# eggsbenedicto/DiffusionRenderer-ComfyUI

Hardware: AMD Instinct MI355X
Metric: denoising_steps_per_sec (higher is better)
Workload: dtype bf16; 1 GPU; inverse pass, 57f x 576 x 1024 clip: EDM Euler step = 1 DiT forward (D=4096, 28 blocks, 32 heads) over S=18432 tokens, guidance 0; parallelism=sp1 (token bands; self-attention exchange: none), weights=random-init (hash generator), 7.2e9 params bf16

## Files before the change

diffusionrenderer-comfyui_amd/csrc/drn_launchers.h:

```cpp
#pragma once
#include "drn_common.h"

struct ConvGeom;

void drn_attention_combine_launch(const float* opart, const float* mlpart, void* o, int nsplit, int batch, int heads, int64_t Sq,
                                  int64_t ldo, int64_t bso, float scale_log2e, void* oq, void* os, int64_t mx_bs, hipStream_t st);
void drn_attention16_launch(const void* q, const void* k, const void* v, void* o, int heads, int64_t Sq, int64_t Sk, int64_t ldq,
                            int64_t ldk, int64_t ldv, int64_t ldo, int64_t bsq, int64_t bsk, int64_t bsv, int64_t bso,
                            float scale_log2e, int nqb, int64_t total, int nsplit, int64_t kv_chunk, float* opart, float* mlpart,
                            hipStream_t st, void* oq, void* os, int64_t mx_bs);

int drn_gemm256s_dispatch(const void* A, const void* W, void* C, int64_t M, int64_t N, int64_t K, int64_t lda, int64_t ldw,
                          int64_t ldc, int epilogue, const void* gate, const void* residual, int64_t ldr, int64_t rpb,
                          void* stream, const int64_t* blk);
int drn_gemm256s_partial(const void* A, const void* W, float* partial, int64_t M, int64_t N, int64_t K, int64_t lda, int64_t ldw,
                         int splits, void* stream, bool wring_ok);
int drn_gemm144_dispatch(const void* A, const void* W, void* C, int64_t M, int64_t N, int64_t K, int64_t lda, int64_t ldw,
                         int64_t ldc, int epilogue, const void* gate, const void* residual, int64_t ldr, int64_t rpb,
                         void* stream, const int64_t* blk);
int drn_gemm_tall_dispatch(const void* A, const void* W, void* C, float* partial, int64_t M, int64_t N, int64_t K, int64_t lda,
                           int64_t ldw, int64_t ldc, int epilogue, const void* gate, const void* residual, int64_t ldr,
                           int64_t rpb, int splits, void* stream);
int drn_gemm_splitk_reduce(const void* workspace, int splits, void* C, int64_t M, int64_t N, int64_t ldc, int epilogue,
                           const void* gate, const void* residual, int64_t ldr, int64_t rows_per_batch, void* stream);
int drn_gemm_mx_gelu_mx_launch(const void* A, const void* SA, const void* W, const void* SW, void* CQ, void* CS, int64_t M, int64_t N,
                               int64_t K, void* stream);

bool drn_conv256s_ok(const ConvGeom& g, int C, int N, int64_t ldc, int64_t ldr, bool has_residual, bool out_f32, const void* y,
                     const void* residual);
int drn_conv256s_launch(const void* x, const void* w, const void* bias, void* y, const void* residual, const ConvGeom& g, int C,
                        int N, int64_t ldw, int64_t ldc, int64_t ldr, void* stream);

struct AttnLaunch {
    int64_t mx_bs;
    int64_t kv_chunk;
    int nsplit;
    int64_t nqb, total;
    float* opart;
    float* mlpart;
    float scale_log2e;
};
static inline int drn_attention_prologue(AttnLaunch* L, void* oq, void* os, bool mx_body, int batch, int heads, int64_t Sq, int64_t Sk,
                                         int64_t ldo, int64_t bso, float scale, int nsplit, void* workspace, int q_rows,
                                         int key_tile) {
    L->mx_bs = 0;
    if (oq) {
        DRN_CHECK_ARG(os && mx_body && ldo == (int64_t)heads * 128 && bso >= 0 && bso % ldo == 0);
        DRN_CHECK_ARG(((uintptr_t)oq & 7) == 0 && ((uintptr_t)os & 3) == 0);
        L->mx_bs = bso / ldo;
        DRN_CHECK_ARG(batch == 1 || L->mx_bs >= Sq);
    }
    L->kv_chunk = Sk;
    L->nsplit = nsplit;
    if (nsplit > 1 && Sq > 0) {
        DRN_CHECK_ARG(workspace && ((uintptr_t)workspace & 15) == 0 && batch <= 65535);
        L->kv_chunk = ((Sk + nsplit - 1) / nsplit + key_tile - 1) / key_tile * key_tile;
        L->nsplit = (int)((Sk + L->kv_chunk - 1) / L->kv_chunk);
    }
    L->nqb = (Sq + q_rows - 1) / q_rows;
    L->total = L->nqb * heads * batch * L->nsplit;
    DRN_CHECK_ARG(L->total < (1ll << 31));
    L->scale_log2e = scale * 1.44269504088896340736f;
    L->opart = (float*)workspace;
    L->mlpart = L->opart ? L->opart + (int64_t)L->nsplit * batch * Sq * heads * 128 : nullptr;
    return DRN_OK;
}
```

diffusionrenderer-comfyui_amd/csrc/gemm.hip:

```cpp
#include <stdlib.h>
#include "drn_common.h"
#include "drn_launchers.h"

#define BM 128
#define BN 128
#define BK 64
#define TILE_BYTES (BM * BK * 2)
#define STAGE_BYTES (2 * TILE_BYTES)

typedef const __attribute__((address_space(1))) void* gptr_t;
typedef __attribute__((address_space(3))) void* lptr_t;

__device__ __forceinline__ float gelu_erf(float x) { return 0.5f * x * (1.0f + erff(x * 0.70710678118654752440f)); }

template <int EPI>
__global__ __launch_bounds__(256, 2) void gemm_bf16_kernel(const bf16_t* __restrict__ A, const bf16_t* __restrict__ W,
                                                           bf16_t* C, int64_t M, int64_t N, int64_t K, int64_t lda,
                                                           int64_t ldw, int64_t ldc, const bf16_t* __restrict__ gate,
                                                           const bf16_t* R, int64_t ldr, int64_t rpb,
                                                           float* __restrict__ part) {
    __shared__ __attribute__((aligned(1024))) char smem[2 * STAGE_BYTES];

    const int tid = threadIdx.x;
    const int lane = tid & 63;
// ... 124 lines not shown
                    for (int r = 0; r < 4; ++r) v[r] = x[r] + rbf(g[r] * v[r]);
                }
                o[h].x = pack_bf2(v[0], v[1]);
                o[h].y = pack_bf2(v[2], v[3]);
            }
            const auto sx = __builtin_amdgcn_permlane16_swap(o[0].x, o[1].x, false, false);
            const auto sy = __builtin_amdgcn_permlane16_swap(o[0].y, o[1].y, false, false);
            const int64_t n8 = n0 + wn * 64 + jp * 32 + (fq & 1) * 16 + (fq >> 1) * 8;
            if (m_ok) *reinterpret_cast<uint4*>(C + m * ldc + n8) = make_uint4(sx[0], sy[0], sx[1], sy[1]);
        }
    }
}

template <int EPI>
__global__ __launch_bounds__(256) void gemm_splitk_epilogue_kernel(const float* __restrict__ part, int splits, bf16_t* C,
                                                                   int64_t M, int64_t N, int64_t ldc,
                                                                   const bf16_t* __restrict__ gate, const bf16_t* R,
                                                                   int64_t ldr, int64_t rpb) {
    const int64_t nq = N / 4, total = M * nq;
    for (int64_t i = (int64_t)blockIdx.x * 256 + threadIdx.x; i < total; i += (int64_t)gridDim.x * 256) {
        const int64_t m = i / nq, n = (i - m * nq) * 4;
        f32x4_t a = *reinterpret_cast<const f32x4_t*>(part + m * N + n);
        for (int s = 1; s < splits; ++s) a += *reinterpret_cast<const f32x4_t*>(part + ((int64_t)s * M + m) * N + n);
        float v[4];
#pragma unroll
        for (int r = 0; r < 4; ++r) v[r] = rbf(a[r]);
        if (EPI == DRN_EPI_GELU) {
#pragma unroll
            for (int r = 0; r < 4; ++r) v[r] = gelu_erf_fast(v[r]);
        } else if (EPI == DRN_EPI_GATE_RES) {
            const uint2 g2 = *reinterpret_cast<const uint2*>(gate + (m / rpb) * N + n);
            const uint2 r2 = *reinterpret_cast<const uint2*>(R + m * ldr + n);
            const float g[4] = {bflo(g2.x), bfhi(g2.x), bflo(g2.y), bfhi(g2.y)};
            const float x[4] = {bflo(r2.x), bfhi(r2.x), bflo(r2.y), bfhi(r2.y)};
#pragma unroll
            for (int r = 0; r < 4; ++r) v[r] = x[r] + rbf(g[r] * v[r]);
        }
        uint2 o;
        o.x = pack_bf2(v[0], v[1]);
        o.y = pack_bf2(v[2], v[3]);
        *reinterpret_cast<uint2*>(C + m * ldc + n) = o;
    }
}

static int g_force_tile = -1;
extern "C" void drn_gemm_force_tile(int tile) { g_force_tile = tile; }
static int tall_choice(int64_t M, int64_t N, int64_t K);

static int pick_gemm_tile(int64_t M, int64_t N, double* cost_out = nullptr) {
    static int mode256 = -1, mode144 = -1;
    static double cost144 = 0.0;
    if (mode256 < 0) {
        const char* e = getenv("DRN_GEMM256");
        mode256 = (e && e[0] == '0') ? 0 : 1;
        e = getenv("DRN_GEMM144");
        mode144 = e ? atoi(e) : 1;
        e = getenv("DRN_GEMM144_COST");
        cost144 = e ? atof(e) : 0.64;
    }
    if (cost_out) *cost_out = 1e30;
    if (N < 256 || N % 256 != 0) return 0;
    if (g_force_tile >= 0) return g_force_tile;
    const int64_t t256 = ((M + 255) / 256) * (N / 256), t128 = ((M + 127) / 128) * (N / 128), t144 = ((M + 143) / 144) * (N / 256);
    const double c128 = 0.65 * (double)((t128 + 511) / 512);
    const double c256 = (mode256 == 1 && M >= 256) ? (double)((t256 + 255) / 256) : 1e30;
    const double c144 = (mode144 >= 1 && M >= 144 && t144 >= 192) ? cost144 * (double)((t144 + 255) / 256) : 1e30;
    if (mode144 == 2 && M >= 144) return 2;
    const int best = (c144 < c256 && c144 < c128) ? 2 : (c256 <= c128 ? 1 : 0);
    if (cost_out) *cost_out = best == 2 ? c144 : (best == 1 ? c256 : c128);
    return best;
}

extern "C" int drn_gemm_tile_choice(int64_t M, int64_t N) { return pick_gemm_tile(M, N); }

static const int64_t kPlain[4] = {62, 0, 62, 0};

static int gemm_launch_tile(int tile, const void* A, const void* W, void* C, int64_t M, int64_t N, int64_t K, int64_t lda,
                            int64_t ldw, int64_t ldc, int epilogue, const void* gate, const void* residual, int64_t ldr,
                            int64_t rows_per_batch, void* stream, const int64_t* blk) {
    if (tile == 1 || tile == 3 || tile == 4)
        return drn_gemm256s_dispatch(A, W, C, M, N, K, lda, ldw, ldc, epilogue, gate, residual, ldr, rows_per_batch, stream, blk);
    if (tile == 2)
        return drn_gemm144_dispatch(A, W, C, M, N, K, lda, ldw, ldc, epilogue, gate, residual, ldr, rows_per_batch, stream, blk);
    const int64_t tiles = ((M + BM - 1) / BM) * (N / BN);
    DRN_CHECK_ARG(tiles < (1ll << 31));
    dim3 grid((unsigned)tiles), block(256);
    hipStream_t st = (hipStream_t)stream;
#define ARGS (const bf16_t*)A, (const bf16_t*)W, (bf16_t*)C, M, N, K, lda, ldw, ldc, (const bf16_t*)gate, \
             (const bf16_t*)residual, ldr, rows_per_batch, (float*)nullptr
    switch (epilogue) {
        case DRN_EPI_NONE: gemm_bf16_kernel<DRN_EPI_NONE><<<grid, block, 0, st>>>(ARGS); break;
        case DRN_EPI_GELU: gemm_bf16_kernel<DRN_EPI_GELU><<<grid, block, 0, st>>>(ARGS); break;
        case DRN_EPI_GATE_RES: gemm_bf16_kernel<DRN_EPI_GATE_RES><<<grid, block, 0, st>>>(ARGS); break;
        default: return DRN_EINVAL;
    }
#undef ARGS
    return drn_launch_status();
}

static int64_t gemm_plan_rows(int64_t M, int64_t N, bool blocked, int* tile_out) {
    double cost_all = 0.0;
    const int tile = pick_gemm_tile(M, N, &cost_all);
    *tile_out = tile;
    static int tail_mode = -1;
    if (tail_mode < 0) {
        const char* e = getenv("DRN_GEMM_TAIL");
        tail_mode = (e && e[0] == '0') ? 0 : 1;
    }
    if (tile != 1 || tail_mode != 1 || g_force_tile >= 0) return M;
    const int64_t tm = (M + 255) / 256, tn = N / 256;
    const int64_t rounds = tm * tn / 256, rem = tm * tn % 256;
    const int64_t tm_main = rounds * 256 / tn;
    if (rounds < 1 || rem == 0 || tm_main < 1 || tm_main >= tm) return M;
    const int64_t M_main = tm_main * 256;
    double cost_tail = 0.0;
    const int tail_tile = pick_gemm_tile(M - M_main, N, &cost_tail);
    if (blocked && tail_tile == 0) cost_tail = 1e30;
    const double cost_split = (double)((tm_main * tn + 255) / 256) + cost_tail + 0.02;
    return cost_split < cost_all - 0.05 ? M_main : M;
}

static int gemm_clip(const void* A, const void* W, void* C, int64_t M, int64_t N, int64_t K, int64_t lda, int64_t ldw,
                     int64_t ldc, int epilogue, const void* gate, const void* residual, int64_t ldr, void* stream,
                     const int64_t* blk) {
    const bool blocked = blk[0] != 62 || blk[2] != 62;
    int tile = 0;
    const int64_t M_main = gemm_plan_rows(M, N, blocked, &tile);
    if (blocked && tile == 0) return DRN_EINVAL;
    if (M_main == M)
        return gemm_launch_tile(tile, A, W, C, M, N, K, lda, ldw, ldc, epilogue, gate, residual, ldr, M, stream, blk);
    const int rc = gemm_launch_tile(1, A, W, C, M_main, N, K, lda, ldw, ldc, epilogue, gate, residual, ldr, M_main, stream, blk);
    if (rc != DRN_OK) return rc;
    return gemm_clip((const bf16_t*)A + M_main * lda, W, (bf16_t*)C + M_main * ldc, M - M_main, N, K, lda, ldw, ldc, epilogue, gate,
                     residual ? (const bf16_t*)residual + M_main * ldr : nullptr, ldr, stream, blk);
}

static int gemm_impl(const void* A, const void* W, void* C, int64_t M, int64_t N, int64_t K, int64_t lda,
                     int64_t ldw, int64_t ldc, int epilogue, const void* gate, const void* residual,
                     int64_t ldr, int64_t rows_per_batch, void* stream, const int64_t* blk) {
    DRN_CHECK_ARG(A && W && C && M >= 0 && N > 0 && K > 0);
    DRN_CHECK_ARG(K % BK == 0 && N % BN == 0);
    DRN_CHECK_ARG(lda % 8 == 0 && ldw % 8 == 0 && ldc % 8 == 0 && ldw >= K);
    DRN_CHECK_ARG((blk[0] != 62 || lda >= K) && (blk[2] != 62 || ldc >= N));
    DRN_CHECK_ARG(((uintptr_t)A & 15) == 0 && ((uintptr_t)W & 15) == 0 && ((uintptr_t)C & 15) == 0);
    if (epilogue == DRN_EPI_GATE_RES)
        DRN_CHECK_ARG(gate && residual && ldr % 8 == 0 && ldr >= N && rows_per_batch > 0 && ((uintptr_t)residual & 7) == 0);
    if (M == 0) return DRN_OK;
    if (epilogue < DRN_EPI_NONE || epilogue > DRN_EPI_GATE_RES) return DRN_EINVAL;
    const bool batched = rows_per_batch > 0 && rows_per_batch < M && M % rows_per_batch == 0 && blk[0] == 62 && blk[2] == 62;
    if (blk[0] == 62 && blk[2] == 62 && M % 256 == 0 && lda >= K && tall_choice(batched ? rows_per_batch : M, N, K) == 1)
        return drn_gemm_tall_dispatch(A, W, C, nullptr, M, N, K, lda, ldw, ldc, epilogue, gate, residual, ldr,
                                      rows_per_batch > 0 ? rows_per_batch : M, 1, stream);
    if (!batched) {
        if (epilogue == DRN_EPI_GATE_RES && rows_per_batch < M) {
            int tile = 0;
            const bool blocked = blk[0] != 62 || blk[2] != 62;
            (void)gemm_plan_rows(M, N, blocked, &tile);
            if (blocked && tile == 0) return DRN_EINVAL;
            return gemm_launch_tile(tile, A, W, C, M, N, K, lda, ldw, ldc, epilogue, gate, residual, ldr, rows_per_batch, stream, blk);
        }
        return gemm_clip(A, W, C, M, N, K, lda, ldw, ldc, epilogue, gate, residual, ldr, stream, blk);
    }
    const int64_t Mb = rows_per_batch, nb = M / Mb;
    int tile = 0;
    if (gemm_plan_rows(Mb, N, false, &tile) == Mb)
        return gemm_launch_tile(tile, A, W, C, M, N, K, lda, ldw, ldc, epilogue, gate, residual, ldr, Mb, stream, blk);
    for (int64_t b = 0; b < nb; ++b) {
        const int rc = gemm_clip((const bf16_t*)A + b * Mb * lda, W, (bf16_t*)C + b * Mb * ldc, Mb, N, K, lda, ldw, ldc, epilogue,
                                 epilogue == DRN_EPI_GATE_RES ? (const bf16_t*)gate + b * N : nullptr,
                                 residual ? (const bf16_t*)residual + b * Mb * ldr : nullptr, ldr, stream, blk);
        if (rc != DRN_OK) return rc;
    }
    return DRN_OK;
}

extern "C" int drn_gemm_bf16(const void* A, const void* W, void* C, int64_t M, int64_t N, int64_t K, int64_t lda,
                             int64_t ldw, int64_t ldc, int epilogue, const void* gate, const void* residual,
                             int64_t ldr, int64_t rows_per_batch, void* stream) {
    return gemm_impl(A, W, C, M, N, K, lda, ldw, ldc, epilogue, gate, residual, ldr, rows_per_batch, stream, kPlain);
}

static int log2_exact(int64_t v) {
    int s = 0;
    while ((1ll << s) < v) ++s;
    return (1ll << s) == v ? s : -1;
}

extern "C" int drn_gemm_bf16_blocked(const void* A, const void* W, void* C, int64_t M, int64_t N, int64_t K, int64_t lda,
                                     int64_t ldw, int64_t ldc, int epilogue, const void* gate, const void* residual,
                                     int64_t ldr, int64_t rows_per_batch, int64_t a_block_cols, int64_t a_block_stride,
                                     int64_t c_block_cols, int64_t c_block_stride, void* stream) {
    int64_t blk[4] = {62, 0, 62, 0};
    if (a_block_cols) {
        const int sh = log2_exact(a_block_cols);
        DRN_CHECK_ARG(sh >= 6 && K % a_block_cols == 0 && a_block_stride % 8 == 0 && lda >= a_block_cols);
        blk[0] = sh;
        blk[1] = a_block_stride;
    }
    if (c_block_cols) {
        const int sh = log2_exact(c_block_cols);
        DRN_CHECK_ARG(sh >= 8 && N % c_block_cols == 0 && c_block_stride % 8 == 0 && ldc >= c_block_cols);
        blk[2] = sh;
        blk[3] = c_block_stride;
    }
    return gemm_impl(A, W, C, M, N, K, lda, ldw, ldc, epilogue, gate, residual, ldr, rows_per_batch, stream, blk);
}

extern "C" int64_t drn_gemm_splitk_workspace_bytes(int64_t M, int64_t N, int splits) {
    return splits > 1 ? (int64_t)splits * M * N * (int64_t)sizeof(float) : 0;
}

static int tall_choice(int64_t M, int64_t N, int64_t K) {
    static int mode = -1;
    if (mode < 0) {
        const char* e = getenv("DRN_GEMM_TALL");
        mode = (e && e[0] == '0') ? 0 : 1;
    }
    if (!mode || g_force_tile >= 0 || M != 256 || N % 64 != 0 || K % BK != 0) return 0;
    const int64_t tiles = N / 64;
    if (tiles >= 192) return 1;
    for (int s = 2; s <= 8; s *= 2)
        if (tiles * s >= 192 && tiles * s <= 256 && (K / BK) % s == 0 && K / s >= 1024 && K / s <= 2048) return s;
    return 0;
}

static int splitk256_choice(int64_t M, int64_t N, int64_t K) {
    static int mode = -1;
    if (mode < 0) {
        const char* e = getenv("DRN_SPLITK256");
        mode = (e && e[0] == '0') ? 0 : 1;
    }
    if (!mode || M % 256 != 0 || N % 256 != 0 || K % BK != 0 || M > 1024) return 0;
    const int64_t tiles = (M / 256) * (N / 256);
    int best = 0;
    for (int s = 2; s <= 16; s *= 2)
        if (tiles * s <= 256 && (K / BK) % s == 0 && K / s >= 1024) best = s;
    return (best && tiles * best >= 192) ? best : 0;
}

extern "C" int drn_gemm_splitk_choice(int64_t M, int64_t N, int64_t K) {
    if (N % BN != 0 || K % BK != 0 || M <= 0) return 1;
    {
        const int st = tall_choice(M, N, K);
        if (st) return st;
    }
    if (g_force_tile < 0 || g_force_tile == 4) {
        const int s256 = splitk256_choice(M, N, K);
        if (s256) return s256;
// ... 76 lines not shown
```

diffusionrenderer-comfyui_amd/native.py:

```python
import ctypes
import os
from ctypes import POINTER, Structure, c_char_p, c_double, c_float, c_int, c_int32, c_int64, c_void_p

import torch

_LIB = None
_LIB_NAME = "libdrn.so"

EPI_NONE, EPI_GELU, EPI_GATE_RES = 0, 1, 2
ACT_NONE, ACT_SILU = 0, 1

_P, _I, _L, _F = c_void_p, c_int, c_int64, c_float

SUB_FA, SUB_CA, SUB_MLP = 0, 1, 2


class DitSub(Structure):
    _fields_ = [("kind", c_int32), ("site", c_int32), ("ca_index", c_int32), ("reserved", c_int32),
                ("w_a", c_void_p), ("w_b", c_void_p), ("qn", c_void_p), ("kn", c_void_p),
                ("s_a", c_void_p), ("s_b", c_void_p)]


class DitForwardArgs(Structure):
    _fields_ = [("struct_bytes", c_int64), ("S", c_int64), ("B", c_int64), ("D", c_int64), ("hidden", c_int64),
                ("heads", c_int32), ("n_sub", c_int32), ("subs", POINTER(DitSub)),
                ("shift", c_void_p), ("scale", c_void_p), ("gate", c_void_p),
                ("shift_site_stride", c_int64), ("scale_site_stride", c_int64), ("gate_site_stride", c_int64),
                ("addvec", c_void_p), ("addvec_stride", c_int64), ("cos", c_void_p), ("sin", c_void_p),
                ("P", c_void_p), ("kpad", c_int64), ("w_patch", c_void_p),
                ("final_shift", c_void_p), ("final_scale", c_void_p), ("w_final", c_void_p), ("n_final", c_int64),
                ("X", c_void_p), ("H", c_void_p), ("QKV", c_void_p), ("O", c_void_p), ("U", c_void_p), ("Y", c_void_p),
                ("gemm_ws", c_void_p), ("gemm_ws_bytes", c_int64), ("attn_ws", c_void_p), ("attn_ws_bytes", c_int64),
                ("timer", c_void_p), ("eps", c_float), ("precision", c_int32),
                ("AQ", c_void_p), ("AS", c_void_p), ("act_bytes", c_int64),
                ("mx_fused", c_int32), ("reserved", c_int32), ("UQ", c_void_p), ("US", c_void_p), ("u_act_bytes", c_int64),
                ("attn_precision", c_int32), ("reserved2", c_int32), ("mx_attn", c_void_p), ("mx_attn_bytes", c_int64)]


SIGNATURES = {
    "drn_attention_plan": [_I, _L, _L, POINTER(c_int64)],
    "drn_dit_forward": [POINTER(DitForwardArgs), _P],
    "drn_dit_forward_args_bytes": [],
    "drn_dit_sub_bytes": [],
    "drn_dit_forward_gemm_workspace_bytes": [_L, _L, _L, _L, _L, _L],
    "drn_dit_forward_attn_workspace_bytes": [_L, _I, _L],
    "drn_dit_forward_mx_act_bytes": [_L, _L, _L, _L],
    "drn_dit_forward_mx_gemm_workspace_bytes": [_L, _L, _L, _L],
    "drn_dit_forward_mx_u_bytes": [_L, _L, _L],
    "drn_timer_create": [_I, _I],
    "drn_timer_destroy": [_P],
    "drn_timer_count": [_P],
    "drn_timer_seen": [_P, _I],
    "drn_timer_read": [_P, _I, POINTER(c_int), POINTER(c_float), POINTER(c_double), POINTER(c_double)],
    "drn_abi_version": [],
    "drn_error_string": [_I],
    "drn_gemm_bf16": [_P, _P, _P, _L, _L, _L, _L, _L, _L, _I, _P, _P, _L, _L, _P],
    "drn_gemm_bf16_blocked": [_P, _P, _P, _L, _L, _L, _L, _L, _L, _I, _P, _P, _L, _L, _L, _L, _L, _L, _P],
    "drn_gemm_bf16_splitk": [_P, _P, _P, _L, _L, _L, _L, _L, _L, _I, _P, _P, _L, _L, _I, _P, _P],
    "drn_gemm_splitk_workspace_bytes": [_L, _L, _I],
    "drn_gemm_bf16_f32out": [_P, _P, _P, _L, _L, _L, _L, _L, _P],
    "drn_gemm_bf16_splitk_partials": [_P, _P, _L, _L, _L, _L, _L, _L, _I, _P, _P],
    "drn_splitk_gate_res_ln_modulate": [_P, _I, _P, _P, _P, _P, _P, _P, _L, _L, _L, _F, _P],
    "drn_gemm_splitk_choice": [_L, _L, _L],
    "drn_gemm_tile_choice": [_L, _L],
    "drn_gemm_force_tile": [_I],
    "drn_gemm_force_res_prefetch": [_I],
    "drn_gemm_tall_force_shape": [_I],
    "drn_mx_quant_bf16": [_P, _L, _L, _L, _P, _P, _P],
    "drn_mx_quant_calls": [_I],
    "drn_gemm_mxfp8_gelu_mx": [_P, _P, _P, _P, _P, _P, _L, _L, _L, _L, _P],
    "drn_ln_modulate_mx": [_P, _P, _P, _P, _P, _P, _P, _L, _L, _L, _F, _P],
    "drn_splitk_gate_res_ln_modulate_mx": [_P, _I, _P, _P, _P, _P, _P, _P, _P, _P, _L, _L, _L, _F, _P],
    "drn_attention_bf16_mx": [_P, _P, _P, _P, _P, _P, _I, _I, _L, _L, _L, _L, _L, _L, _L, _L, _L, _L, _F, _P],
    "drn_attention_splitkv_bf16_mx": [_P, _P, _P, _P, _P, _P, _I, _I, _L, _L, _L, _L, _L, _L, _L, _L, _L, _L, _F, _I, _P, _P],
    "drn_attention_mx_available": [],
    "drn_attention_mxfp8_params": [POINTER(c_int), POINTER(c_float), POINTER(c_int)],
    "drn_attention_mxfp8_choice": [_I, _L],
    "drn_attention_mxfp8_force": [_I],
    "drn_qk_norm_rope_mx": [_P, _P, _P, _P, _P, _P, _P, _P, _P, _P, _L, _I, _L, _L, _L, _L, _F, _I, _P],
    "drn_mx_quant_vt": [_P, _P, _P, _I, _I, _L, _L, _L, _P],
    "drn_attention_mxfp8": [_P, _P, _P, _P, _P, _P, _P, _P, _P, _I, _I, _L, _L, _L, _L, _L, _L, _F, _P],
    "drn_attention_splitkv_mxfp8": [_P, _P, _P, _P, _P, _P, _P, _P, _P, _I, _I, _L, _L, _L, _L, _L, _L, _F, _I, _P, _P],
    "drn_dit_forward_mx_attn_bytes": [_L, _L, _L],
    "drn_dit_forward_mx_attn_layout": [_L, _L, _L, POINTER(c_int64)],
    "drn_gemm_mxfp8": [_P, _P, _P, _P, _P, _L, _L, _L, _L, _I, _P, _P, _L, _L, _P],
    "drn_gemm_mxfp8_blocked": [_P, _P, _P, _P, _P, _L, _L, _L, _L, _I, _P, _P, _L, _L, _L, _L, _L, _L, _P],
    "drn_gemm_mxfp8_splitk_choice": [_L, _L, _L],
    "drn_gemm_mxfp8_splitk": [_P, _P, _P, _P, _P, _L, _L, _L, _L, _I, _P, _P, _L, _L, _I, _P, _P],
    "drn_gemm_mxfp8_splitk_partials": [_P, _P, _P, _P, _L, _L, _L, _L, _I, _P, _P],
    "drn_gemm_mxfp8_force_small_m": [_I],
    "drn_gemm_mxfp8_tall_force_shape": [_I],
    "drn_gemv_bf16": [_P, _P, _P, _L, _L, _I, _I, _L, _L, _L, _L, _L, _P, _L, _L, _P, _L, _L, _I, _P],
    "drn_ln_modulate": [_P, _P, _P, _P, _P, _L, _L, _L, _F, _P],
    "drn_ln_force_kernel": [_I],
    "drn_bcast_add": [_P, _P, _L, _L, _L, _P],
    "drn_permute_021": [_P, _P, _L, _L, _L, _P],
    "drn_rmsnorm": [_P, _P, _P, _L, _L, _F, _P],
    "drn_qk_norm_rope": [_P, _P, _P, _P, _P, _P, _L, _I, _L, _L, _L, _L, _F, _P],
    "drn_attention_bf16": [_P, _P, _P, _P, _I, _I, _L, _L, _L, _L, _L, _L, _L, _L, _L, _L, _F, _P],
    "drn_attention_splitkv_bf16": [_P, _P, _P, _P, _I, _I, _L, _L, _L, _L, _L, _L, _L, _L, _L, _L, _F, _I, _P, _P],
    "drn_attention_splitkv_workspace_bytes": [_I, _I, _L, _I],
    "drn_attention_force_shape16": [_I],
    "drn_patchify_concat": [_P, _P, _P, _I, _I, _I, _I, _I, _I, _I, _I, _I, _L, _P],
    "drn_unpatchify": [_P, _L, _P, _I, _I, _I, _I, _I, _I, _I, _P],
    "drn_edm_scale_input": [_P, _P, _L, _F, _P],
    "drn_edm_step": [_P, _P, _P, _L, _F, _F, _F, _F, _P],
    "drn_cfg_combine": [_P, _P, _P, _L, _F, _P],
    "drn_postprocess_u8": [_P, _P, _I, _I, _I, _I, _I, _P],
    "drn_postprocess_window_u8": [_P, _P, _P, _P, _I, _I, _I, _I, _I, _I, _I, _I, _I, _P],
    "drn_env_project": [_P, _I, _P, _P, _P, _P, _I, _I, _I, _F, _P],
    "drn_fit_frames": [_P, _P, _I, _I, _I, _I, _I, _I, _I, _P, _P, _P, _I, _P, _P, _I, _P],
    "drn_fit_frames_u8": [_P, _P, _I, _I, _I, _I, _I, _I, _I, _P, _P, _P, _I, _P, _P, _I, _P],
    "drn_restore_frames_u8": [_P, _P, _I, _I, _I, _I, _I, _I, _I, _P, _P, _I, _P, _P, _I, _P],
    "drn_restore_guided_u8": [_P, _P, _P, _P, _I, _I, _I, _I, _I, _I, _I, _I, _I, _I, _P, _P, _I, _P, _P, _I, _P, _F, _P],
    "drn_tile_blend_u8": [_P, _P, _P, _P, _L, _I, _I, _I, _I, _I, _I, _I, _I, _I, _I, _P],
    "drn_latent_tile_gather": [_P, _P, _L, _I, _I, _I, _I, _I, _I, _F, _I, _P],
    "drn_latent_tile_step_join": [_P, _P, _F, _P, _P, _P, _P, _L, _I, _I, _I, _I, _I, _I, _I, _I, _I, _I, _F, _F, _F, _F, _P],
}
_RESTYPES = {"drn_error_string": c_char_p, "drn_attention_splitkv_workspace_bytes": c_int64,
             "drn_gemm_splitk_workspace_bytes": c_int64, "drn_dit_forward_gemm_workspace_bytes": c_int64,
             "drn_dit_forward_attn_workspace_bytes": c_int64, "drn_dit_forward_mx_act_bytes": c_int64,
             "drn_dit_forward_mx_u_bytes": c_int64, "drn_mx_quant_calls": c_int64, "drn_dit_forward_mx_attn_bytes": c_int64,
             "drn_dit_forward_mx_gemm_workspace_bytes": c_int64, "drn_dit_forward_args_bytes": c_int64, "drn_dit_sub_bytes": c_int64, "drn_timer_create": c_void_p, "drn_timer_destroy": None,
             "drn_ln_force_kernel": None, "drn_attention_force_shape16": None}


def library_path() -> str:
    return os.path.join(os.path.dirname(os.path.abspath(__file__)), _LIB_NAME)


def load_library():
    global _LIB
    if _LIB is not None:
        return _LIB
    path = library_path()
    if not os.path.exists(path):
        raise RuntimeError(f"{path} not found: build it with `python __graft_entry__.py` (hipcc --offload-arch=gfx950); "
                           "there is no CPU / eager fallback for the hot path")
    lib = ctypes.CDLL(path)
    for name, argtypes in SIGNATURES.items():
        fn = getattr(lib, name)
        fn.argtypes = argtypes
        fn.restype = _RESTYPES.get(name, c_int)
    if lib.drn_abi_version() != 1:
        raise RuntimeError("libdrn.so ABI version mismatch")
    if lib.drn_dit_forward_args_bytes() != ctypes.sizeof(DitForwardArgs) or lib.drn_dit_sub_bytes() != ctypes.sizeof(DitSub):
        raise RuntimeError("libdrn.so: drn_dit_forward_args / drn_dit_sub layout differs from the ctypes mirror in native.py")
    _LIB = lib
# ... 759 lines not shown
```

include/drn.h:

```cpp
#ifndef DRN_H
#define DRN_H

#include <stdint.h>

#ifdef __cplusplus
extern "C" {
#endif

#define DRN_OK 0
#define DRN_EINVAL (-1)

#define DRN_ABI_VERSION 1

#define DRN_EPI_NONE 0
#define DRN_EPI_GELU 1
#define DRN_EPI_GATE_RES 2

#define DRN_ACT_NONE 0
#define DRN_ACT_SILU 1

int drn_abi_version(void);
const char* drn_error_string(int code);

int drn_gemm_bf16(const void* A, const void* W, void* C, int64_t M, int64_t N, int64_t K,
                  int64_t lda, int64_t ldw, int64_t ldc, int epilogue,
                  const void* gate, const void* residual, int64_t ldr, int64_t rows_per_batch,
                  void* stream);

int drn_gemm_bf16_blocked(const void* A, const void* W, void* C, int64_t M, int64_t N, int64_t K,
                          int64_t lda, int64_t ldw, int64_t ldc, int epilogue,
                          const void* gate, const void* residual, int64_t ldr, int64_t rows_per_batch,
                          int64_t a_block_cols, int64_t a_block_stride, int64_t c_block_cols, int64_t c_block_stride,
                          void* stream);

int drn_gemm_bf16_splitk(const void* A, const void* W, void* C, int64_t M, int64_t N, int64_t K,
                         int64_t lda, int64_t ldw, int64_t ldc, int epilogue,
                         const void* gate, const void* residual, int64_t ldr, int64_t rows_per_batch,
                         int splits, void* workspace, void* stream);
int64_t drn_gemm_splitk_workspace_bytes(int64_t M, int64_t N, int splits);
int drn_gemm_bf16_f32out(const void* A, const void* W, float* C, int64_t M, int64_t N, int64_t K, int64_t lda, int64_t ldw, void* stream);

int drn_gemm_bf16_splitk_partials(const void* A, const void* W, int64_t M, int64_t N, int64_t K,
                                  int64_t lda, int64_t ldw, int64_t rows_per_batch, int splits, void* workspace, void* stream);
int drn_gemm_splitk_choice(int64_t M, int64_t N, int64_t K);

int drn_gemm_tile_choice(int64_t M, int64_t N);
void drn_gemm_force_tile(int tile);
int drn_gemm_force_res_prefetch(int on);
int drn_gemm_tall_force_shape(int shape);

int drn_mx_quant_bf16(const void* X, int64_t M, int64_t K, int64_t ldx, void* Q, void* scales, void* stream);
int64_t drn_mx_quant_calls(int reset);
int drn_gemm_mxfp8_gelu_mx(const void* A, const void* SA, const void* W, const void* SW, void* CQ, void* CS, int64_t M, int64_t N,
                           int64_t K, int64_t rows_per_batch, void* stream);
int drn_gemm_mxfp8(const void* A, const void* SA, const void* W, const void* SW, void* C, int64_t M, int64_t N, int64_t K,
                   int64_t ldc, int epilogue, const void* gate, const void* residual, int64_t ldr, int64_t rows_per_batch,
                   void* stream);
int drn_gemm_mxfp8_blocked(const void* A, const void* SA, const void* W, const void* SW, void* C, int64_t M, int64_t N, int64_t K,
                           int64_t ldc, int epilogue, const void* gate, const void* residual, int64_t ldr, int64_t rows_per_batch,
                           int64_t a_block_cols, int64_t a_block_stride, int64_t c_block_cols, int64_t c_block_stride,
                           void* stream);
int drn_gemm_mxfp8_splitk_choice(int64_t M, int64_t N, int64_t K);
int drn_gemm_mxfp8_splitk(const void* A, const void* SA, const void* W, const void* SW, void* C, int64_t M, int64_t N, int64_t K,
                          int64_t ldc, int epilogue, const void* gate, const void* residual, int64_t ldr, int64_t rows_per_batch,
                          int splits, void* workspace, void* stream);
int drn_gemm_mxfp8_splitk_partials(const void* A, const void* SA, const void* W, const void* SW, int64_t M, int64_t N, int64_t K,
                                   int64_t rows_per_batch, int splits, void* workspace, void* stream);
int drn_gemm_mxfp8_force_small_m(int on);
int drn_gemm_mxfp8_tall_force_shape(int shape);

int drn_gemv_bf16(const void* x, const void* W, void* y, int64_t N, int64_t K,
                  int groups, int batch,
                  int64_t x_gstride, int64_t x_bstride, int64_t w_gstride,
                  int64_t y_gstride, int64_t y_bstride,
                  const void* add, int64_t add_gstride, int64_t add_bstride,
                  const void* mul, int64_t mul_gstride, int64_t mul_bstride,
                  int act, void* stream);

int drn_ln_modulate(void* x, const void* add_vec, const void* shift, const void* scale, void* h,
                    int64_t rows, int64_t D, int64_t rows_per_batch, float eps, void* stream);
int drn_ln_modulate_mx(void* x, const void* add_vec, const void* shift, const void* scale, void* h, void* hq, void* hs,
                       int64_t rows, int64_t D, int64_t rows_per_batch, float eps, void* stream);
int drn_splitk_gate_res_ln_modulate(const void* partials, int splits, void* x, const void* gate, const void* add_vec,
                                    const void* shift, const void* scale, void* h, int64_t rows, int64_t D,
                                    int64_t rows_per_batch, float eps, void* stream);
int drn_splitk_gate_res_ln_modulate_mx(const void* partials, int splits, void* x, const void* gate, const void* add_vec,
                                       const void* shift, const void* scale, void* h, void* hq, void* hs, int64_t rows, int64_t D,
                                       int64_t rows_per_batch, float eps, void* stream);
void drn_ln_force_kernel(int which);

int drn_bcast_add(void* x, const void* vec, int64_t rows, int64_t D, int64_t rows_per_batch, void* stream);

int drn_permute_021(const void* x, void* y, int64_t A, int64_t B, int64_t C, void* stream);

int drn_rmsnorm(const void* x, const void* w, void* y, int64_t rows, int64_t D, float eps, void* stream);

int drn_qk_norm_rope(void* q, void* k, const void* wq, const void* wk, const void* cos, const void* sin,
                     int64_t tokens, int heads, int64_t ldq, int64_t ldk, int64_t tokens_per_batch,
                     int64_t pos_offset, float eps, void* stream);

int drn_attention_bf16(const void* q, const void* k, const void* v, void* o,
                       int batch, int heads, int64_t Sq, int64_t Sk,
                       int64_t ldq, int64_t ldk, int64_t ldv, int64_t ldo,
                       int64_t bsq, int64_t bsk, int64_t bsv, int64_t bso,
                       float scale, void* stream);

void drn_attention_force_shape16(int on);

int drn_attention_splitkv_bf16(const void* q, const void* k, const void* v, void* o,
                               int batch, int heads, int64_t Sq, int64_t Sk,
                               int64_t ldq, int64_t ldk, int64_t ldv, int64_t ldo,
                               int64_t bsq, int64_t bsk, int64_t bsv, int64_t bso,
                               float scale, int nsplit, void* workspace, void* stream);
int64_t drn_attention_splitkv_workspace_bytes(int batch, int heads, int64_t Sq, int nsplit);

int drn_attention_bf16_mx(const void* q, const void* k, const void* v, void* o, void* oq, void* os,
                          int batch, int heads, int64_t Sq, int64_t Sk,
                          int64_t ldq, int64_t ldk, int64_t ldv, int64_t ldo,
                          int64_t bsq, int64_t bsk, int64_t bsv, int64_t bso,
                          float scale, void* stream);
int drn_attention_splitkv_bf16_mx(const void* q, const void* k, const void* v, void* o, void* oq, void* os,
                                  int batch, int heads, int64_t Sq, int64_t Sk,
                                  int64_t ldq, int64_t ldk, int64_t ldv, int64_t ldo,
                                  int64_t bsq, int64_t bsk, int64_t bsv, int64_t bso,
                                  float scale, int nsplit, void* workspace, void* stream);
int drn_attention_mx_available(void);

int drn_attention_mxfp8_params(int* key_tile, float* rescale_thr, int* pexp);
int drn_attention_mxfp8_choice(int heads, int64_t S);
int drn_attention_mxfp8_force(int on);
// ... 155 lines not shown
```

Baseline: 3.693 steps/s.

## Add 384x256 bf16 GEMM kernel with scheduled MFMA/DMA pipeline for FFN down-projection

Adds a new large-tile (384x256x64) bf16 GEMM kernel with a hand-interleaved MFMA schedule, direct global-to-LDS loads and double-buffered stages, split across VGPR and AGPR accumulators. The tile planner picks it for an allow-listed shape (18432x4096x16384, the FFN down-projection) when its wave-quantized cost is no worse than the existing tiles. The larger tile raises arithmetic intensity per LDS byte and reduces operand traffic. The cost is one wave per SIMD, a heavy register footprint, and possible tail-wave imbalance.

```diff
diff --git a/diffusionrenderer-comfyui_amd/csrc/drn_launchers.h b/diffusionrenderer-comfyui_amd/csrc/drn_launchers.h
--- a/diffusionrenderer-comfyui_amd/csrc/drn_launchers.h
+++ b/diffusionrenderer-comfyui_amd/csrc/drn_launchers.h
@@ -15,6 +15,10 @@
                           void* stream, const int64_t* blk);
 int drn_gemm256s_partial(const void* A, const void* W, float* partial, int64_t M, int64_t N, int64_t K, int64_t lda, int64_t ldw,
                          int splits, void* stream, bool wring_ok);
+bool drn_gemm384_ok(int64_t M, int64_t N, int64_t K, int64_t ldmax, int epilogue, int64_t rpb, const int64_t* blk);
+int drn_gemm384_dispatch(const void* A, const void* W, void* C, int64_t M, int64_t N, int64_t K, int64_t lda, int64_t ldw,
+                         int64_t ldc, int epilogue, const void* gate, const void* residual, int64_t ldr, int64_t rpb,
+                         void* stream, const int64_t* blk);
 int drn_gemm144_dispatch(const void* A, const void* W, void* C, int64_t M, int64_t N, int64_t K, int64_t lda, int64_t ldw,
                          int64_t ldc, int epilogue, const void* gate, const void* residual, int64_t ldr, int64_t rpb,
                          void* stream, const int64_t* blk);
diff --git a/diffusionrenderer-comfyui_amd/csrc/gemm.hip b/diffusionrenderer-comfyui_amd/csrc/gemm.hip
--- a/diffusionrenderer-comfyui_amd/csrc/gemm.hip
+++ b/diffusionrenderer-comfyui_amd/csrc/gemm.hip
@@ -230,6 +230,8 @@
         return drn_gemm256s_dispatch(A, W, C, M, N, K, lda, ldw, ldc, epilogue, gate, residual, ldr, rows_per_batch, stream, blk);
     if (tile == 2)
         return drn_gemm144_dispatch(A, W, C, M, N, K, lda, ldw, ldc, epilogue, gate, residual, ldr, rows_per_batch, stream, blk);
+    if (tile == 5)
+        return drn_gemm384_dispatch(A, W, C, M, N, K, lda, ldw, ldc, epilogue, gate, residual, ldr, rows_per_batch, stream, blk);
     const int64_t tiles = ((M + BM - 1) / BM) * (N / BN);
     DRN_CHECK_ARG(tiles < (1ll << 31));
     dim3 grid((unsigned)tiles), block(256);
@@ -246,10 +248,11 @@
     return drn_launch_status();
 }
 
-static int64_t gemm_plan_rows(int64_t M, int64_t N, bool blocked, int* tile_out) {
+static int64_t gemm_plan_rows256(int64_t M, int64_t N, bool blocked, int* tile_out, double* cost_out) {
     double cost_all = 0.0;
     const int tile = pick_gemm_tile(M, N, &cost_all);
     *tile_out = tile;
+    *cost_out = cost_all;
     static int tail_mode = -1;
     if (tail_mode < 0) {
         const char* e = getenv("DRN_GEMM_TAIL");
@@ -265,7 +268,54 @@
     const int tail_tile = pick_gemm_tile(M - M_main, N, &cost_tail);
     if (blocked && tail_tile == 0) cost_tail = 1e30;
     const double cost_split = (double)((tm_main * tn + 255) / 256) + cost_tail + 0.02;
-    return cost_split < cost_all - 0.05 ? M_main : M;
+    if (cost_split < cost_all - 0.05) {
+        *cost_out = cost_split;
+        return M_main;
+    }
+    return M;
+}
+
+struct Gemm384Shape { int64_t M, N, K; };
+static const Gemm384Shape kGemm384Measured[] = {
+    {18432, 4096, 16384},
+};
+static bool gemm384_choice(int64_t M, int64_t N, int64_t K, int64_t ldmax, bool blocked, double cost_today) {
+    static int mode = -1;
+    if (mode < 0) {
+        const char* e = getenv("DRN_GEMM384");
+        mode = e ? atoi(e) : 1;
+        if (mode < 0 || mode > 2) mode = 1;
+    }
+    if (!mode || g_force_tile >= 0 || blocked) return false;
+    if (!drn_gemm384_ok(M, N, K, ldmax, DRN_EPI_GATE_RES, M, nullptr)) return false;
+    const int64_t t384 = (M / 384) * (N / 256);
+    const double cost384 = 1.5 * (double)((t384 + 255) / 256);
+    if (t384 % 256 != 0 && !(cost384 < cost_today)) return false;
+    if (mode == 2) return true;
+    for (const Gemm384Shape& s : kGemm384Measured)
+        if (s.M == M && s.N == N && s.K == K) return true;
+    return false;
+}
+
+static int64_t gemm_plan_rows(int64_t M, int64_t N, int64_t K, int64_t ldmax, bool blocked, int* tile_out) {
+    double cost_today = 0.0;
+    const int64_t M_main = gemm_plan_rows256(M, N, blocked, tile_out, &cost_today);
+    if (gemm384_choice(M, N, K, ldmax, blocked, cost_today)) {
+        *tile_out = 5;
+        return M;
+    }
+    return M_main;
+}
+
+extern "C" int drn_gemm_plan_choice(int64_t M, int64_t N, int64_t K, int64_t rows_per_batch, int64_t* main_rows) {
+    if (main_rows) *main_rows = 0;
+    if (M <= 0 || N <= 0 || K <= 0 || N % BN != 0 || K % BK != 0) return DRN_EINVAL;
+    const bool batched = rows_per_batch > 0 && rows_per_batch < M && M % rows_per_batch == 0;
+    const int64_t Mb = batched ? rows_per_batch : M;
+    int tile = 0;
+    const int64_t rows = gemm_plan_rows(Mb, N, K, N > K ? N : K, false, &tile);
+    if (main_rows) *main_rows = rows;
+    return tile;
 }
 
 static int gemm_clip(const void* A, const void* W, void* C, int64_t M, int64_t N, int64_t K, int64_t lda, int64_t ldw,
@@ -273,7 +323,10 @@
                      const int64_t* blk) {
     const bool blocked = blk[0] != 62 || blk[2] != 62;
     int tile = 0;
-    const int64_t M_main = gemm_plan_rows(M, N, blocked, &tile);
+    int64_t ldmax = lda > ldw ? lda : ldw;
+    if (ldc > ldmax) ldmax = ldc;
+    if (residual && ldr > ldmax) ldmax = ldr;
+    const int64_t M_main = gemm_plan_rows(M, N, K, ldmax, blocked, &tile);
     if (blocked && tile == 0) return DRN_EINVAL;
     if (M_main == M)
         return gemm_launch_tile(tile, A, W, C, M, N, K, lda, ldw, ldc, epilogue, gate, residual, ldr, M, stream, blk);
@@ -303,7 +356,8 @@
         if (epilogue == DRN_EPI_GATE_RES && rows_per_batch < M) {
             int tile = 0;
             const bool blocked = blk[0] != 62 || blk[2] != 62;
-            (void)gemm_plan_rows(M, N, blocked, &tile);
+            double cost = 0.0;
+            (void)gemm_plan_rows256(M, N, blocked, &tile, &cost);
             if (blocked && tile == 0) return DRN_EINVAL;
             return gemm_launch_tile(tile, A, W, C, M, N, K, lda, ldw, ldc, epilogue, gate, residual, ldr, rows_per_batch, stream, blk);
         }
@@ -311,7 +365,10 @@
     }
     const int64_t Mb = rows_per_batch, nb = M / Mb;
     int tile = 0;
-    if (gemm_plan_rows(Mb, N, false, &tile) == Mb)
+    int64_t ldmax = lda > ldw ? lda : ldw;
+    if (ldc > ldmax) ldmax = ldc;
+    if (residual && ldr > ldmax) ldmax = ldr;
+    if (gemm_plan_rows(Mb, N, K, ldmax, false, &tile) == Mb)
         return gemm_launch_tile(tile, A, W, C, M, N, K, lda, ldw, ldc, epilogue, gate, residual, ldr, Mb, stream, blk);
     for (int64_t b = 0; b < nb; ++b) {
         const int rc = gemm_clip((const bf16_t*)A + b * Mb * lda, W, (bf16_t*)C + b * Mb * ldc, Mb, N, K, lda, ldw, ldc, epilogue,
diff --git a/diffusionrenderer-comfyui_amd/csrc/gemm384.hip b/diffusionrenderer-comfyui_amd/csrc/gemm384.hip
--- /dev/null
+++ b/diffusionrenderer-comfyui_amd/csrc/gemm384.hip
@@ -0,0 +1,319 @@
+#include <stdlib.h>
+#include "drn_common.h"
+#include "drn_launchers.h"
+
+#define G384_BM 384
+#define G384_BN 256
+#define G384_BK 64
+#define G384_AH (192 * G384_BK * 2)
+#define G384_WH (128 * G384_BK * 2)
+#define G384_STAGE (2 * G384_AH + 2 * G384_WH)
+#define G384_LDS (2 * G384_STAGE)
+#define G384_A(S, I) ((S) * G384_STAGE + (I) * G384_AH)
+#define G384_W(S, J) ((S) * G384_STAGE + 2 * G384_AH + (J) * G384_WH)
+
+typedef const __attribute__((address_space(1))) void* g384_gptr_t;
+typedef __attribute__((address_space(3))) void* g384_lptr_t;
+
+static __device__ __forceinline__ void tile_of384(int bid, int nwg, int tiles_m, int tiles_n, int GROUP, int64_t& m0, int64_t& n0) {
+    const int q = nwg >> 3, r = nwg & 7, xcd = bid & 7;
+    const int pid = (xcd < r ? xcd * (q + 1) : r * (q + 1) + (xcd - r) * q) + (bid >> 3);
+    const int width = GROUP * tiles_n;
+    const int group_id = pid / width;
+    const int first_m = group_id * GROUP;
+    const int gsz = min(tiles_m - first_m, GROUP);
+    m0 = (int64_t)(first_m + (pid % width) % gsz) * G384_BM;
+    n0 = (int64_t)((pid % width) / gsz) * G384_BN;
+}
+
+#define FENCE() __builtin_amdgcn_sched_barrier(0)
+#define LDA(S, I, MT, KS) (*reinterpret_cast<const bf16x8_t*>(smem + G384_A(S, I) + offa[KS] + (MT) * 2048))
+#define LDW(S, J, NT, KS) (*reinterpret_cast<const bf16x8_t*>(smem + G384_W(S, J) + offw[KS] + (NT) * 2048))
+static __device__ __forceinline__ void g384_dma16(const char* sbase, uint32_t voff, uint32_t dst) {
+    uint32_t keep;
+    asm volatile("s_mov_b32 %0, m0\n\ts_mov_b32 m0, %3\n\ts_nop 0\n\tglobal_load_lds_dwordx4 %1, %2\n\ts_mov_b32 m0, %0"
+                 : "=&s"(keep) : "v"(voff), "s"(sbase), "s"(dst) : "memory");
+}
+#define DMA_A(I, P, BASE, S) g384_dma16(BASE, voffa[P], lds0 + G384_A(S, I) + (P) * 4096 + dma_off)
+#define DMA_W(J, P, BASE, S) g384_dma16(BASE, voffw[P], lds0 + G384_W(S, J) + (P) * 4096 + dma_off)
+#define G384_IN_V(I, MT, J) ((I) == 1 && ((J) == 0 || (MT) < 2))
+#define MM(I, MT, J, NT, WF)                                                                                           \
+    do {                                                                                                               \
+        if (G384_IN_V(I, MT, J))                                                                                       \
+            asm volatile("v_mfma_f32_16x16x32_bf16 %0, %1, %2, %0" : "+v"(acc[I][MT][J][NT]) : "v"(WF[NT]), "v"(af[MT])); \
+        else                                                                                                           \
+            asm volatile("v_mfma_f32_16x16x32_bf16 %0, %1, %2, %0" : "+a"(acc[I][MT][J][NT]) : "v"(WF[NT]), "v"(af[MT])); \
+    } while (0)
+#define SLOT_M(I, J, MT, WF, WORK)                                                                                     \
+    do {                                                                                                               \
+        MM(I, MT, J, 0, WF); MM(I, MT, J, 1, WF); MM(I, MT, J, 2, WF); MM(I, MT, J, 3, WF);                            \
+        WORK;                                                                                                          \
+        FENCE();                                                                                                       \
+    } while (0)
+#define SLOT_N(I, J, NT, WF, WORK)                                                                                     \
+    do {                                                                                                               \
+        MM(I, 0, J, NT, WF); MM(I, 1, J, NT, WF); MM(I, 2, J, NT, WF);                                                 \
+        MM(I, 3, J, NT, WF); MM(I, 4, J, NT, WF); MM(I, 5, J, NT, WF);                                                 \
+        WORK;                                                                                                          \
+        FENCE();                                                                                                       \
+    } while (0)
+#define HANDOVER(VM)                                                                                                   \
+    do {                                                                                                               \
+        FENCE();                                                                                                       \
+        asm volatile("s_waitcnt vmcnt(" #VM ")" ::: "memory");                                                         \
+        __builtin_amdgcn_s_barrier();                                                                                  \
+        FENCE();                                                                                                       \
+    } while (0)
+#define HANDOVER_B()                          \
+    do {                                                                                                               \
+        FENCE();                                                                                                       \
+        __builtin_amdgcn_s_barrier();                                                                                  \
+        FENCE();                                                                                                       \
+    } while (0)
+#define HANDOVER_N() FENCE()
+#define HSTEP(S, KS, SN, KSN, WA, WB, DW, DA, H1, H2, H3, H4)                                                          \
+    do {                                                                                                               \
+                                                                                 \
+        SLOT_M(0, 0, 0, WA, WB[0] = LDW(S, 1, 0, KS));                                                                 \
+        SLOT_M(0, 0, 1, WA, WB[1] = LDW(S, 1, 1, KS));                                                                 \
+        SLOT_M(0, 0, 2, WA, WB[2] = LDW(S, 1, 2, KS));                                                                 \
+        SLOT_M(0, 0, 3, WA, WB[3] = LDW(S, 1, 3, KS));                                                                 \
+        SLOT_M(0, 0, 4, WA, DW(0));                                                                                    \
+        SLOT_M(0, 0, 5, WA, DW(1));                                                                                    \
+        H1;                                                                                                            \
+                                                                  \
+        SLOT_M(0, 1, 0, WB, af[0] = LDA(S, 1, 0, KS));                                                                 \
+        SLOT_M(0, 1, 1, WB, (af[1] = LDA(S, 1, 1, KS), DW(2)));                                                        \
+        SLOT_M(0, 1, 2, WB, af[2] = LDA(S, 1, 2, KS));                                                                 \
+        SLOT_M(0, 1, 3, WB, (af[3] = LDA(S, 1, 3, KS), DW(3)));                                                        \
+        SLOT_M(0, 1, 4, WB, af[4] = LDA(S, 1, 4, KS));                                                                 \
+        SLOT_M(0, 1, 5, WB, af[5] = LDA(S, 1, 5, KS));                                                                 \
+        H2;                                                                                                            \
+                            \
+        SLOT_N(1, 1, 0, WB, (WB[0] = LDW(SN, 0, 0, KSN), DA(0)));                                                      \
+        SLOT_N(1, 1, 1, WB, (WB[1] = LDW(SN, 0, 1, KSN), DA(1)));                                                      \
+        SLOT_N(1, 1, 2, WB, (WB[2] = LDW(SN, 0, 2, KSN), DA(2)));                                                      \
+        SLOT_N(1, 1, 3, WB, WB[3] = LDW(SN, 0, 3, KSN));                                                               \
+        H3;                                                                                                            \
+                                            \
+        SLOT_M(1, 0, 0, WA, af[0] = LDA(SN, 0, 0, KSN));                                                               \
+        SLOT_M(1, 0, 1, WA, (af[1] = LDA(SN, 0, 1, KSN), DA(3)));                                                      \
+        SLOT_M(1, 0, 2, WA, af[2] = LDA(SN, 0, 2, KSN));                                                               \
+        SLOT_M(1, 0, 3, WA, (af[3] = LDA(SN, 0, 3, KSN), DA(4)));                                                      \
+        SLOT_M(1, 0, 4, WA, af[4] = LDA(SN, 0, 4, KSN));                                                               \
+        SLOT_M(1, 0, 5, WA, (af[5] = LDA(SN, 0, 5, KSN), DA(5)));                                                      \
+        H4;                                                                                                            \
+    } while (0)
+#define KSTEP(S, KD1, KD2)                                                                                             \
+    do {                                                                                                               \
+        HSTEP(S, 0, S, 1, wx, wy, DW_1, DA_1, HANDOVER(12), HANDOVER_N(), HANDOVER_N(), HANDOVER_B());                 \
+        HSTEP(S, 1, (S) ^ 1, 0, wy, wx, DW_0, DA_0, HANDOVER_N(), HANDOVER(20), HANDOVER(17), HANDOVER(16));           \
+    } while (0)
+
+template <int EPI, int I, int J>
+static __device__ __forceinline__ void store_quarter384(f32x4_t (&acc)[2][6][2][4], bf16_t* C, int64_t N, int64_t ldc,
+                                                        const bf16_t* __restrict__ gate, const bf16_t* R, int64_t ldr,
+                                                        int64_t rpb, int64_t m0, int64_t n0, int wr, int wc, int fr, int fq) {
+    const int row = I * 192 + wr * 96 + fr;
+    char* cbase = reinterpret_cast<char*>(C + m0 * ldc + n0);
+    const uint32_t coff = (uint32_t)((row * (int)ldc + J * 128 + wc * 64 + (fq & 1) * 16 + (fq >> 1) * 8) * 2);
+    uint2 g2[4], r2[6][4];
+    if (EPI == DRN_EPI_GATE_RES) {
+        const int64_t b = (int64_t)((uint32_t)m0 / (uint32_t)rpb);
+        const char* gbase = reinterpret_cast<const char*>(gate + b * N + n0);
+        const char* rbase = reinterpret_cast<const char*>(R + m0 * ldr + n0);
+        const uint32_t goff = (uint32_t)((J * 128 + wc * 64 + fq * 4) * 2);
+        const uint32_t roff = (uint32_t)((row * (int)ldr) * 2) + goff;
+#pragma unroll
+        for (int nt = 0; nt < 4; ++nt) {
+            g2[nt] = *reinterpret_cast<const uint2*>(gbase + (goff + (uint32_t)(nt * 32)));
+#pragma unroll
+            for (int mt = 0; mt < 6; ++mt)
+                r2[mt][nt] = *reinterpret_cast<const uint2*>(rbase + (roff + (uint32_t)(mt * 16 * (int)ldr * 2) + (uint32_t)(nt * 32)));
+        }
+    }
+#pragma unroll
+    for (int mt = 0; mt < 6; ++mt)
+#pragma unroll
+        for (int q = 0; q < 2; ++q) {
+            uint2 o[2];
+#pragma unroll
+            for (int h = 0; h < 2; ++h) {
+                const int nt = 2 * q + h;
+                float v[4];
+#pragma unroll
+                for (int r = 0; r < 4; ++r) v[r] = rbf(acc[I][mt][J][nt][r]);
+                if (EPI == DRN_EPI_GELU) {
+#pragma unroll
+                    for (int r = 0; r < 4; ++r) v[r] = gelu_erf_fast(v[r]);
+                } else if (EPI == DRN_EPI_GATE_RES) {
+                    const uint2 gg = g2[nt], rr = r2[mt][nt];
+                    const float g[4] = {bflo(gg.x), bfhi(gg.x), bflo(gg.y), bfhi(gg.y)};
+                    const float x[4] = {bflo(rr.x), bfhi(rr.x), bflo(rr.y), bfhi(rr.y)};
+#pragma unroll
+                    for (int r = 0; r < 4; ++r) v[r] = x[r] + rbf(g[r] * v[r]);
+                }
+                o[h].x = pack_bf2(v[0], v[1]);
+                o[h].y = pack_bf2(v[2], v[3]);
+            }
+            const auto sx = __builtin_amdgcn_permlane16_swap(o[0].x, o[1].x, false, false);
+            const auto sy = __builtin_amdgcn_permlane16_swap(o[0].y, o[1].y, false, false);
+            const u32x4_t val = {sx[0], sy[0], sx[1], sy[1]};
+            *reinterpret_cast<u32x4_t*>(cbase + (coff + (uint32_t)(mt * 16 * (int)ldc * 2) + (uint32_t)(q * 64))) = val;
+        }
+}
+
+template <int EPI>
+__global__ __launch_bounds__(256) __attribute__((amdgpu_waves_per_eu(1, 1)))
+void gemm384_kernel(const bf16_t* __restrict__ A, const bf16_t* __restrict__ W, bf16_t* C, int64_t M, int64_t N, int64_t K,
+                    int64_t lda, int64_t ldw, int64_t ldc, const bf16_t* __restrict__ gate, const bf16_t* R, int64_t ldr,
+                    int64_t rpb, int GROUP) {
+    extern __shared__ __attribute__((aligned(1024))) char smem[];
+    const int tid = threadIdx.x;
+    const int lane = tid & 63;
+    const int wave = __builtin_amdgcn_readfirstlane(tid >> 6);
+    const int wr = wave >> 1, wc = wave & 1;
+    const int tiles_m = (int)(M / G384_BM), tiles_n = (int)(N / G384_BN);
+    const int nk = (int)(K / G384_BK);
+    int64_t m0, n0;
+    tile_of384(blockIdx.x, tiles_m * tiles_n, tiles_m, tiles_n, GROUP, m0, n0);
+    const int dma_off = wave * 1024;
+    const uint32_t lds0 = (uint32_t)(uintptr_t)(g384_lptr_t)smem;
+    const int fr = lane & 15, fq = lane >> 4;
+    int offa[2], offw[2];
+    {
+        const int ra = wr * 96 + fr;
+        const int rw = wc * 64 + fr;
+        offa[0] = ra * 128 + ((fq ^ ((ra >> 1) & 7)) << 4);
+        offw[0] = rw * 128 + ((fq ^ ((rw >> 1) & 7)) << 4);
+        offa[1] = offa[0] ^ 64;
+        offw[1] = offw[0] ^ 64;
+    }
+    const char* abase = reinterpret_cast<const char*>(A + m0 * lda);
+    const char* wbase = reinterpret_cast<const char*>(W + n0 * ldw);
+    uint32_t voffa[6], voffw[4];
+    {
+        const int r = wave * 8 + (lane >> 3);
+        const int c = (lane & 7) ^ ((r >> 1) & 7);
+#pragma unroll
+        for (int p = 0; p < 6; ++p) voffa[p] = (uint32_t)(((r + 32 * p) * (int)lda + c * 8) * 2);
+#pragma unroll
+        for (int p = 0; p < 4; ++p) voffw[p] = (uint32_t)(((r + 32 * p) * (int)ldw + c * 8) * 2);
+    }
+    const int64_t a1off = 192 * lda * 2, w1off = 128 * ldw * 2;
+    f32x4_t acc[2][6][2][4];
+    bf16x8_t af[6], wx[4], wy[4];
+#pragma unroll
+    for (int i = 0; i < 2; ++i)
+#pragma unroll
+        for (int mt = 0; mt < 6; ++mt)
+#pragma unroll
+            for (int j = 0; j < 2; ++j)
+#pragma unroll
+                for (int nt = 0; nt < 4; ++nt) acc[i][mt][j][nt] = (f32x4_t){0.f, 0.f, 0.f, 0.f};
+
+#pragma unroll
+    for (int p = 0; p < 4; ++p) DMA_W(0, p, wbase, 0);
+#pragma unroll
+    for (int p = 0; p < 6; ++p) DMA_A(0, p, abase, 0);
+#pragma unroll
+    for (int p = 0; p < 4; ++p) DMA_W(1, p, wbase + w1off, 0);
+#pragma unroll
+    for (int p = 0; p < 6; ++p) DMA_A(1, p, abase + a1off, 0);
+#pragma unroll
+    for (int p = 0; p < 4; ++p) DMA_W(0, p, wbase + 2 * G384_BK, 1);
+#pragma unroll
+    for (int p = 0; p < 6; ++p) DMA_A(0, p, abase + 2 * G384_BK, 1);
+    asm volatile("s_waitcnt vmcnt(20)" ::: "memory");
+    __builtin_amdgcn_s_barrier();
+    FENCE();
+#pragma unroll
+    for (int nt = 0; nt < 4; ++nt) wx[nt] = LDW(0, 0, nt, 0);
+#pragma unroll
+    for (int mt = 0; mt < 6; ++mt) af[mt] = LDA(0, 0, mt, 0);
+    FENCE();
+    asm volatile("s_waitcnt vmcnt(16)" ::: "memory");
+    __builtin_amdgcn_s_barrier();
+    FENCE();
+#define DW_1(P) DMA_W(1, P, wbase + w1off + (int64_t)kd1 * (2 * G384_BK), sn)
+#define DA_1(P) DMA_A(1, P, abase + a1off + (int64_t)kd1 * (2 * G384_BK), sn)
+#define DW_0(P) DMA_W(0, P, wbase + (int64_t)kd2 * (2 * G384_BK), sc)
+#define DA_0(P) DMA_A(0, P, abase + (int64_t)kd2 * (2 * G384_BK), sc)
+    int kt = 0;
+    for (; kt + 1 < nk; kt += 2) {
+        {
+            const int kd1 = kt + 1, kd2 = min(kt + 2, nk - 1);
+            constexpr int sc = 0, sn = 1;
+            KSTEP(0, kd1, kd2);
+        }
+        {
+            const int kd1 = min(kt + 2, nk - 1), kd2 = min(kt + 3, nk - 1);
+            constexpr int sc = 1, sn = 0;
+            KSTEP(1, kd1, kd2);
+        }
+    }
+    if (kt < nk) {
+        const int kd1 = nk - 1, kd2 = nk - 1;
+        constexpr int sc = 0, sn = 1;
+        KSTEP(0, kd1, kd2);
+    }
+    asm volatile("s_waitcnt vmcnt(0)\n\ts_nop 15\n\ts_nop 15" ::: "memory");
+    int efr = fr, efq = fq;
+    asm volatile("" : "+v"(efr), "+v"(efq));
+    store_quarter384<EPI, 1, 0>(acc, C, N, ldc, gate, R, ldr, rpb, m0, n0, wr, wc, efr, efq);
+    store_quarter384<EPI, 1, 1>(acc, C, N, ldc, gate, R, ldr, rpb, m0, n0, wr, wc, efr, efq);
+    store_quarter384<EPI, 0, 0>(acc, C, N, ldc, gate, R, ldr, rpb, m0, n0, wr, wc, efr, efq);
+    store_quarter384<EPI, 0, 1>(acc, C, N, ldc, gate, R, ldr, rpb, m0, n0, wr, wc, efr, efq);
+}
+
+template <int EPI>
+static int launch384(const void* A, const void* W, void* C, int64_t M, int64_t N, int64_t K, int64_t lda, int64_t ldw,
+                     int64_t ldc, const void* gate, const void* residual, int64_t ldr, int64_t rpb, hipStream_t st) {
+    static bool configured = false;
+    if (!configured) {
+        hipError_t e = hipFuncSetAttribute(reinterpret_cast<const void*>(&gemm384_kernel<EPI>),
+                                           hipFuncAttributeMaxDynamicSharedMemorySize, G384_LDS);
+        if (e != hipSuccess) return (int)e;
+        configured = true;
+    }
+    static int group = 0;
+    if (group == 0) {
+        const char* e = getenv("DRN_GEMM_GROUP");
+        group = e ? atoi(e) : 4;
+        if (group < 1) group = 4;
+    }
+    const int64_t tiles = (M / G384_BM) * (N / G384_BN);
+    gemm384_kernel<EPI><<<dim3((unsigned)tiles), dim3(256), G384_LDS, st>>>(
+        (const bf16_t*)A, (const bf16_t*)W, (bf16_t*)C, M, N, K, lda, ldw, ldc, (const bf16_t*)gate, (const bf16_t*)residual, ldr,
+        rpb, group);
+    return drn_launch_status();
+}
+
+bool drn_gemm384_ok(int64_t M, int64_t N, int64_t K, int64_t ldmax, int epilogue, int64_t rpb, const int64_t* blk) {
+    if (blk && (blk[0] != 62 || blk[2] != 62)) return false;
+    if (M < G384_BM || M % G384_BM != 0 || N % G384_BN != 0 || K % G384_BK != 0 || K < 2 * G384_BK) return false;
+    if (M >= (1ll << 31) || (M / G384_BM) * (N / G384_BN) >= (1ll << 31)) return false;
+    if (ldmax < K || (G384_BM * ldmax + 4096) * 2 >= (1ll << 31)) return false;
+    if (epilogue == DRN_EPI_GATE_RES) {
+        if (rpb <= 0 || rpb > M) rpb = M;
+        if (rpb % G384_BM != 0) return false;
+    }
+    return true;
+}
+
+int drn_gemm384_dispatch(const void* A, const void* W, void* C, int64_t M, int64_t N, int64_t K, int64_t lda, int64_t ldw,
+                         int64_t ldc, int epilogue, const void* gate, const void* residual, int64_t ldr, int64_t rpb,
+                         void* stream, const int64_t* blk) {
+    int64_t ldmax = lda > ldw ? lda : ldw;
+    if (ldc > ldmax) ldmax = ldc;
+    if (epilogue == DRN_EPI_GATE_RES && ldr > ldmax) ldmax = ldr;
+    if (lda < K || ldw < K || !drn_gemm384_ok(M, N, K, ldmax, epilogue, rpb, blk)) return DRN_EINVAL;
+    if (rpb > M || rpb <= 0) rpb = M;
+    hipStream_t st = (hipStream_t)stream;
+    switch (epilogue) {
+        case DRN_EPI_NONE: return launch384<DRN_EPI_NONE>(A, W, C, M, N, K, lda, ldw, ldc, gate, residual, ldr, rpb, st);
+        case DRN_EPI_GELU: return launch384<DRN_EPI_GELU>(A, W, C, M, N, K, lda, ldw, ldc, gate, residual, ldr, rpb, st);
+        case DRN_EPI_GATE_RES: return launch384<DRN_EPI_GATE_RES>(A, W, C, M, N, K, lda, ldw, ldc, gate, residual, ldr, rpb, st);
+        default: return DRN_EINVAL;
+    }
+}
diff --git a/diffusionrenderer-comfyui_amd/native.py b/diffusionrenderer-comfyui_amd/native.py
--- a/diffusionrenderer-comfyui_amd/native.py
+++ b/diffusionrenderer-comfyui_amd/native.py
@@ -64,6 +64,7 @@
     "drn_gemm_splitk_choice": [_L, _L, _L],
     "drn_gemm_tile_choice": [_L, _L],
     "drn_gemm_force_tile": [_I],
+    "drn_gemm_plan_choice": [_L, _L, _L, _L, _P],
     "drn_gemm_force_res_prefetch": [_I],
     "drn_gemm_tall_force_shape": [_I],
     "drn_mx_quant_bf16": [_P, _L, _L, _L, _P, _P, _P],
diff --git a/include/drn.h b/include/drn.h
--- a/include/drn.h
+++ b/include/drn.h
@@ -46,6 +46,7 @@
 
 int drn_gemm_tile_choice(int64_t M, int64_t N);
 void drn_gemm_force_tile(int tile);
+int drn_gemm_plan_choice(int64_t M, int64_t N, int64_t K, int64_t rows_per_batch, int64_t* main_rows);
 int drn_gemm_force_res_prefetch(int on);
 int drn_gemm_tall_force_shape(int shape);
 
```

Result: faster. 3.737 steps/s, median of 6 (+1.2%).
